# ReaganCardoza/Physics-Based-Ray-Tracing

Hardware: AMD Instinct MI355X
Metric: Msamples/s on cbox.xml 512x512 x 256 spp (radiance, path max_depth 6) (higher is better)
Workload: dtype f32

## Files before the change

### physics-based-ray-tracing_amd/csrc/kernels_radiance.h

```cpp
#pragma once
#include "device_scene.h"
#include "render_request.h"
#include "tile_cull.h"

#ifndef SEG_BRUTE
#define SEG_BRUTE 512
#endif
#ifndef SEG_BVH
#define SEG_BVH 1024
#endif
#ifndef SEG_WAVES_PER_EU
#define SEG_WAVES_PER_EU 8
#endif
#ifndef REGION_SEGS_BVH
#define REGION_SEGS_BVH 4
#endif
#ifndef REGION_SEGS_BRUTE
#define REGION_SEGS_BRUTE 1
#endif
#ifndef REGION_SEGS_US
#define REGION_SEGS_US 8
#endif
__host__ __device__ constexpr uint32_t rad_region_segs(int accel);
#ifndef REGION_SEGS_US_EMIT
// ... 669 lines not shown
#pragma unroll
            for (uint32_t k = 0; k < 2 + MAX_CHAIN; ++k) {
                add[k] = k == 2 ? cnt_in : atomicAdd(&wg_cnt[k < 2 ? k : k - 1], 0u);
                if (k < 2 + nb_run) v[k] = row[k * stride];
            }
#pragma unroll
            for (uint32_t k = 0; k < 2 + MAX_CHAIN; ++k)
                if (k < 2 + nb_run) row[k * stride] = v[k] + add[k];
        }
    }
}

struct TileKeepArgs {
    const pbrt_prim *prims;
    uint32_t n_prims;
    pbrt_camera cam;
    FilmKey key;
    uint32_t n_blocks;
    uint32_t *keep;
};
__global__ __launch_bounds__(64) void k_tile_keep(const TileKeepArgs a) {
    const uint32_t blk = blockIdx.x * 64u + threadIdx.x;
    if (blk >= a.n_blocks) return;
    uint32_t x0 = 0xffffffffu, y0 = 0xffffffffu, x1 = 0, y1 = 0;
    for (uint32_t k = 0; k < 64u; ++k) {
        uint32_t rx, ry;
        region_pixel(a.key, blk * 64u + k, &rx, &ry);
        x0 = min(x0, rx);
        x1 = max(x1, rx);
        y0 = min(y0, ry);
        y1 = max(y1, ry);
    }
    uint32_t word = 0;
    for (uint32_t i = 0; i < a.n_prims && i < 32u; ++i) {
        const pbrt_prim P = load_prim_uniform(a.prims + i);
        if (tile_cull_keep(a.cam, a.key.rx0 + x0, a.key.ry0 + y0, a.key.rx0 + x1, a.key.ry0 + y1, P)) word |= 1u << i;
    }
    word |= a.n_prims < 32u ? ~0u << a.n_prims : 0u;
    a.keep[blk] = word;
}

#define REDUCE_SLICES 32
__global__ __launch_bounds__(256) void k_reduce_stats(const unsigned long long *stats, uint32_t nseg, size_t stride,
                                                      unsigned long long *out) {
    __shared__ unsigned long long part[256];
    const unsigned long long *row = stats + (size_t)blockIdx.x * stride;
    const uint32_t per = (nseg + gridDim.y - 1) / gridDim.y, lo = min(blockIdx.y * per, nseg), hi = min(lo + per, nseg);
    unsigned long long s = 0;
    for (uint32_t i = lo + threadIdx.x; i < hi; i += 256) s += row[i];
    part[threadIdx.x] = s;
    __syncthreads();
    for (uint32_t w = 128; w > 0; w >>= 1) {
        if (threadIdx.x < w) part[threadIdx.x] += part[threadIdx.x + w];
        __syncthreads();
    }
    if (threadIdx.x == 0 && part[0]) atomicAdd(&out[blockIdx.x], part[0]);
}

__global__ __launch_bounds__(256) void k_us_reduce_stats(unsigned long long *stats, uint32_t nseg, size_t stride,
                                                         unsigned long long *out) {
    __shared__ unsigned long long part[4];
    unsigned long long *row = stats + (size_t)blockIdx.x * stride;
    const uint32_t per = (nseg + gridDim.y - 1) / gridDim.y, lo = min(blockIdx.y * per, nseg), hi = min(lo + per, nseg);
    unsigned long long s = 0;
    for (uint32_t i = lo + threadIdx.x; i < hi; i += 256) {
        s += row[i];
        row[i] = 0ull;
    }
#pragma unroll
    for (int off = 32; off > 0; off >>= 1) s += __shfl_xor(s, off);
    if ((threadIdx.x & 63u) == 0u) part[threadIdx.x >> 6] = s;
    __syncthreads();
    if (threadIdx.x == 0) out[(size_t)blockIdx.x * gridDim.y + blockIdx.y] = part[0] + part[1] + part[2] + part[3];
}

struct FilmArgs {
    const float *Lhome;
    float *acc;
    uint32_t cap;
    uint32_t cx0, cy0, cw, ch;
    FilmKey key;
    uint32_t rh;
    uint32_t s_count, filter, seed;
};

DEV float filter_1d(uint32_t f, float x) {
    if (f == PBRT_FILTER_TENT) return fmaxf(0.0f, 1.0f - fabsf(x));
    const float alpha = -2.0f;
    return fmaxf(0.0f, expf(alpha * x * x) - expf(alpha * 4.0f));
}

__global__ __launch_bounds__(256) void k_film_accum(const FilmArgs a) {
    const uint32_t idx = blockIdx.x * blockDim.x + threadIdx.x;
    if (idx >= a.cw * a.ch) return;
    const uint32_t iy = idx / a.cw, ix = idx - iy * a.cw;
    const int x = (int)(a.cx0 + ix), y = (int)(a.cy0 + iy);
    const uint32_t npx = a.cw * a.ch;
    float ar = a.acc[idx], ag = a.acc[npx + idx], ab = a.acc[2 * npx + idx], aw = a.acc[3 * npx + idx];
    const int R = a.filter == PBRT_FILTER_BOX ? 0 : (a.filter == PBRT_FILTER_TENT ? 1 : 2);
    const float ccx = (float)x + 0.5f, ccy = (float)y + 0.5f;
    for (uint32_t sl = 0; sl < a.s_count; ++sl) {
        const uint32_t s_idx = a.key.s_first + sl;
        const float4 *Ls = reinterpret_cast<const float4 *>(a.Lhome) + (size_t)sl * a.key.npix_r;
        for (int ny = y - R; ny <= y + R; ++ny)
            for (int nx = x - R; nx <= x + R; ++nx) {
                if (nx < 0 || ny < 0 || nx >= (int)a.key.film_w || ny >= (int)a.key.film_h) continue;
                float w = 1.0f;
                if (a.filter != PBRT_FILTER_BOX) {
                    F4 uj = rng4((uint32_t)ny * a.key.film_w + (uint32_t)nx, s_idx, 0, a.seed);
                    float px = (float)nx + uj.x, py = (float)ny + uj.y;
                    w = filter_1d(a.filter, ccx - px) * filter_1d(a.filter, ccy - py);
                }
                if (w > 0.0f) {
                    const uint32_t k = region_index((uint32_t)(nx - (int)a.key.rx0), (uint32_t)(ny - (int)a.key.ry0), a.key.rw, a.key.tile_rows);
                    const float4 Lk = Ls[k];
                    ar = fma_(w, Lk.x, ar);
                    ag = fma_(w, Lk.y, ag);
                    ab = fma_(w, Lk.z, ab);
                    aw += w;
                }
            }
    }
    a.acc[idx] = ar;
    a.acc[npx + idx] = ag;
    a.acc[2 * npx + idx] = ab;
    a.acc[3 * npx + idx] = aw;
}

#define FILM_RMAX 2
template <int FILM_TILE, int FILTER>
__global__ __launch_bounds__(FILM_TILE *FILM_TILE) void k_film_accum_tiled(const FilmArgs a) {
    constexpr int FILM_TW = FILM_TILE + 2 * FILM_RMAX;
    constexpr int LS = FILM_TILE == 16 ? 48 : 40;
    static_assert(LS >= FILM_TW, "row stride covers the haloed row");
    __shared__ float tile[2][5][FILM_TW * LS];
    constexpr int R = FILTER == PBRT_FILTER_TENT ? 1 : 2;
    constexpr int TW = FILM_TILE + 2 * R;
    const uint32_t tid = threadIdx.y * FILM_TILE + threadIdx.x;
    const int tx0 = (int)(a.cx0 + blockIdx.x * FILM_TILE), ty0 = (int)(a.cy0 + blockIdx.y * FILM_TILE);
    const int x = tx0 + (int)threadIdx.x, y = ty0 + (int)threadIdx.y;
    const bool inside = x < (int)(a.cx0 + a.cw) && y < (int)(a.cy0 + a.ch);
    const uint32_t npx = a.cw * a.ch;
    const uint32_t idx = inside ? (uint32_t)(y - (int)a.cy0) * a.cw + (uint32_t)(x - (int)a.cx0) : 0u;
    float ar = 0, ag = 0, ab = 0, aw = 0;
    if (inside) {
        ar = a.acc[idx];
        ag = a.acc[npx + idx];
        ab = a.acc[2 * npx + idx];
        aw = a.acc[3 * npx + idx];
    }
    const float ccx = (float)x + 0.5f, ccy = (float)y + 0.5f;
    constexpr int NT = FILM_TILE * FILM_TILE, NST = (FILM_TW * FILM_TW + NT - 1) / NT;
    bool st_in[NST], st_valid[NST];
    uint32_t st_key[NST], st_k[NST];
    float st_x[NST], st_y[NST];
    int st_lds[NST];
#pragma unroll
    for (int j = 0; j < NST; ++j) {
        const int i = (int)tid + j * NT;
        const int nx = tx0 - R + i % TW, ny = ty0 - R + i / TW;
        st_lds[j] = (i / TW) * LS + i % TW;
        st_in[j] = i < TW * TW;
        st_valid[j] = st_in[j] && nx >= (int)a.key.rx0 && ny >= (int)a.key.ry0 && nx < (int)(a.key.rx0 + a.key.rw) && ny < (int)(a.key.ry0 + a.rh);
        st_key[j] = (uint32_t)ny * a.key.film_w + (uint32_t)nx;
        st_k[j] = st_valid[j] ? region_index((uint32_t)(nx - (int)a.key.rx0), (uint32_t)(ny - (int)a.key.ry0), a.key.rw, a.key.tile_rows) : 0u;
        st_x[j] = (float)nx;
        st_y[j] = (float)ny;
    }
    const float4 *Lrec = reinterpret_cast<const float4 *>(a.Lhome);
    const float4 zero4 = {0.0f, 0.0f, 0.0f, 0.0f};
#ifndef FILM_PF
#define FILM_PF 4
#endif
    constexpr int PF = FILM_PF;
    float4 Lq[PF][NST];
#pragma unroll
    for (int u = 0; u < PF; ++u)
#pragma unroll
        for (int j = 0; j < NST; ++j)
            Lq[u][j] = (st_valid[j] && (uint32_t)u < a.s_count) ? Lrec[(size_t)u * a.key.npix_r + st_k[j]] : zero4;
    for (uint32_t sl0 = 0; sl0 < a.s_count; sl0 += PF) {
#pragma unroll
        for (int u = 0; u < PF; ++u) {
            const uint32_t sl = sl0 + (uint32_t)u;
            if (sl >= a.s_count) break;
            const uint32_t s_idx = a.key.s_first + sl;
            float(*T)[FILM_TW * LS] = tile[sl & 1];
#pragma unroll
            for (int j = 0; j < NST; ++j) {
                if (!st_in[j]) continue;
                const int i = st_lds[j];
                float px = 1e30f, py = 1e30f;
                if (st_valid[j]) {
                    F4 uj = rng4(st_key[j], s_idx, 0, a.seed);
                    px = st_x[j] + uj.x;
                    py = st_y[j] + uj.y;
                }
                T[0][i] = px;
                T[1][i] = py;
                T[2][i] = Lq[u][j].x;
                T[3][i] = Lq[u][j].y;
                T[4][i] = Lq[u][j].z;
            }
#pragma unroll
            for (int j = 0; j < NST; ++j)
                Lq[u][j] = (st_valid[j] && sl + PF < a.s_count) ? Lrec[(size_t)(sl + PF) * a.key.npix_r + st_k[j]] : zero4;
            __syncthreads();
            if (inside) {
                const int e0 = (int)threadIdx.y * LS + (int)threadIdx.x;
#pragma unroll
                for (int dy = 0; dy <= 2 * R; ++dy)
#pragma unroll
                    for (int dx = 0; dx <= 2 * R; ++dx) {
                        const int e = e0 + dy * LS + dx;
                        float w = filter_1d(FILTER, ccx - T[0][e]) * filter_1d(FILTER, ccy - T[1][e]);
                        if (w > 0.0f) {
                            ar = fma_(w, T[2][e], ar);
                            ag = fma_(w, T[3][e], ag);
                            ab = fma_(w, T[4][e], ab);
                            aw += w;
                        }
                    }
            }
        }
    }
    if (inside) {
        a.acc[idx] = ar;
        a.acc[npx + idx] = ag;
        a.acc[2 * npx + idx] = ab;
        a.acc[3 * npx + idx] = aw;
    }
}

__global__ __launch_bounds__(256) void k_film_resolve(const float *acc, float *out, uint32_t npx, uint32_t raw) {
    const uint32_t idx = blockIdx.x * blockDim.x + threadIdx.x;
    if (idx >= npx) return;
    float r = acc[idx], g = acc[npx + idx], b = acc[2 * npx + idx], w = acc[3 * npx + idx];
    if (raw) {
        out[4 * idx] = r;
        out[4 * idx + 1] = g;
        out[4 * idx + 2] = b;
        out[4 * idx + 3] = w;
    } else {
        float inv = w > 0.0f ? 1.0f / w : 0.0f;
        out[3 * idx] = r * inv;
        out[3 * idx + 1] = g * inv;
        out[3 * idx + 2] = b * inv;
    }
}

__global__ __launch_bounds__(256) void k_init_rays(float *st, uint32_t *seg_cnt, uint32_t n_cnt, uint32_t region, uint32_t n,
                                                   const float *o, const float *d, const float *tmax) {
    const uint32_t i = blockIdx.x * blockDim.x + threadIdx.x;
    if (i < n_cnt) seg_cnt[i] = n > i * region ? min(n - i * region, region) : 0u;
    if (i >= n) return;
    float *s = st + (state_voff(i) >> 2);
    s[(ST_O + 0) * 64] = o[i];
    s[(ST_O + 1) * 64] = o[n + i];
    s[(ST_O + 2) * 64] = o[2 * n + i];
    s[(ST_D + 0) * 64] = d[i];
    s[(ST_D + 1) * 64] = d[n + i];
    s[(ST_D + 2) * 64] = d[2 * n + i];
    s[(ST_THR + 0) * 64] = 1.0f;
    s[(ST_THR + 1) * 64] = 1.0f;
    s[(ST_THR + 2) * 64] = 1.0f;
    s[(ST_L + 0) * 64] = 0.0f;
    s[(ST_L + 1) * 64] = 0.0f;
    s[(ST_L + 2) * 64] = 0.0f;
    s[ST_ETA * 64] = tmax[i];
    s[ST_PDF * 64] = -1.0f;
    s[ST_HOME * 64] = __uint_as_float(i);
}
```

### physics-based-ray-tracing_amd/csrc/pbrt_api.hip

```cpp
#include <hip/hip_runtime.h>

#include <atomic>
#include <cmath>
#include <cstdarg>
#include <cstdio>
#include <cstring>
#include <map>
#include <numeric>
#include <string>
#include <tuple>
#include <vector>

#include "scene_request.h"
#include "bf_request.h"
#include "us_request.h"
#include "kernels_us.h"
#include "kernels_wavefront.h"
#include "kernels_us_wavefront.h"
#include "kernels_beamform.h"
#ifdef PBRT_DIAG
#include "kernels_diag.h"
#endif
#include "stage_layout.h"
#include "workspace.h"
// ... 844 lines not shown
}
static uint64_t default_pass_paths(pbrt_ctx *c, bool streams, uint64_t paths, uint32_t bytes_per_path) {
    return streams ? wf_default_pass_paths(c) : fused_default_pass_paths(paths, bytes_per_path, c->work.limit);
}

static bool fastdiv_exact(const FastDiv &fd, uint32_t d, std::initializer_list<uint32_t> probes) {
    for (uint32_t n : probes)
        if (udiv_fast(n, fd) != n / d) return false;
    return true;
}

static WfArgs wf_args(const RadArgs &a) {
    WfArgs w{};
    w.sc = a.sc;
    w.cam = a.cam;
    w.Lhome = a.Lhome;
    w.stats = a.stats;
    w.stat_stride = a.stat_stride;
    w.cap = a.cap;
    w.n_paths = a.n_paths;
    w.max_depth = a.max_depth;
    w.rr_depth = a.rr_depth;
    w.seed = a.seed;
    w.key_mode = a.key_mode;
    w.key = a.key;
    w.index_offset = a.index_offset;
    w.sample_index = a.sample_index;
    return w;
}
static void film_accum(pbrt_ctx *c, const FilmArgs &fa) {
    hipStream_t st = c->stream;
    if (fa.filter == PBRT_FILTER_BOX) {
        hipLaunchKernelGGL(k_film_accum, dim3(div_up((uint64_t)fa.cw * fa.ch, 256)), dim3(256), 0, st, fa);
        return;
    }
    const bool big = (uint64_t)div_up(fa.cw, 16) * div_up(fa.ch, 16) >= 4ull * (uint64_t)c->n_cu;
    const bool tent = fa.filter == PBRT_FILTER_TENT;
    const dim3 g16(div_up(fa.cw, 16), div_up(fa.ch, 16)), g8(div_up(fa.cw, 8), div_up(fa.ch, 8));
    if (big && tent)
        hipLaunchKernelGGL((k_film_accum_tiled<16, PBRT_FILTER_TENT>), g16, dim3(16, 16), 0, st, fa);
    else if (big)
        hipLaunchKernelGGL((k_film_accum_tiled<16, PBRT_FILTER_GAUSSIAN>), g16, dim3(16, 16), 0, st, fa);
    else if (tent)
        hipLaunchKernelGGL((k_film_accum_tiled<8, PBRT_FILTER_TENT>), g8, dim3(8, 8), 0, st, fa);
    else
        hipLaunchKernelGGL((k_film_accum_tiled<8, PBRT_FILTER_GAUSSIAN>), g8, dim3(8, 8), 0, st, fa);
}

static int probe_plan(pbrt_ctx *c, unsigned long long *segstats, uint32_t n_rows, uint32_t stat_rows, unsigned long long *dstats,
                      uint32_t max_depth, uint32_t *plan) {
    hipStream_t st = c->stream;
    unsigned long long hp[2 + MAX_DEPTH_STATS];
    hipLaunchKernelGGL(k_reduce_stats, dim3(stat_rows, REDUCE_SLICES), dim3(256), 0, st, segstats, n_rows, (size_t)n_rows, dstats);
    HIPCHK(c, hipGetLastError());
    HIPCHK(c, hipMemcpyAsync(hp, dstats, (size_t)stat_rows * 8, hipMemcpyDeviceToHost, st));
    HIPCHK(c, hipStreamSynchronize(st));
    HIPCHK(c, hipMemsetAsync(dstats, 0, (2 + 2 * MAX_DEPTH_STATS) * 8, st));
    for (uint32_t d = stat_rows; d < 2 + MAX_DEPTH_STATS; ++d) hp[d] = 0;
    *plan = plan_from_survival(hp + 2, std::min<uint32_t>(max_depth, MAX_DEPTH_STATS));
    return PBRT_OK;
}

namespace {
struct Render {
    pbrt_scene *s;
    pbrt_ctx *c;
    const pbrt_camera *cam;
    const pbrt_film_desc *f;
    void *d_out;
    RenderRequest rq;
    Switches sw;
    PassShape ps;
    uint32_t n_own = 0, n_rows = 0;
    WfBufs wfb{};
    WfPlan wfp;
    float *Lhome = nullptr, *acc = nullptr;
    uint32_t *segA = nullptr, *segB = nullptr;
    unsigned long long *dstats = nullptr, *segstats = nullptr;
    FusePlan fp;
    RadArgs base{};
    FilmArgs fa{};
    PassTimer timer{};
    uint32_t passes = 0, launches = 0;
    unsigned long long hstats[2 + 2 * MAX_DEPTH_STATS];
    uint32_t hguard[WF_GUARD_WORDS] = {0};
};
}

static RenderLaunch render_launch(const pbrt_scene *s) {
    static_assert(WF_REGION == REGION_SEGS_BVH * SEG_BVH, "both BVH launch structures cut a pass into the same regions");
    const int k = s->accel_kernel;
    RenderLaunch l;
    l.brute = k == ACCEL_K_BRUTE || k == ACCEL_K_BRUTE_BIG;
    l.keep = k == ACCEL_K_BRUTE && s->ds.n_prims <= 32;
    l.region = rad_region_segs(k) * seg_threads(k);
    l.owners = rad_owners_per_region(k);
    l.rows_fused = k == ACCEL_K_BRUTE ? std::max(rad_rows_per_region(k), path_groups_per_region()) : rad_rows_per_region(k);
    l.rows_streams = WF_SHADE_THREADS / 64u;
    return l;
}

static int render_check(Render &r) {
    pbrt_ctx *c = r.c;
    if (int rcs = ctx_settle(c)) return rcs;
    if (const char *why = render_request(&r.rq, r.cam, r.f, r.d_out != nullptr, render_launch(r.s))) return RULE_TEXT(c, why);
    HIPCHK(c, hipSetDevice(c->device));
    r.sw = read_switches();
    return PBRT_OK;
}

static int render_buffers(Render &r) {
    pbrt_scene *s = r.s;
    pbrt_ctx *c = r.c;
    const pbrt_film_desc *f = r.f;
    const RenderRequest &rq = r.rq;
    const bool wavefront = rq.wavefront;
    const uint64_t pass_paths = f->pass_paths ? f->pass_paths
                                              : default_pass_paths(c, wavefront, rq.brute ? (64u << 20) : (16u << 20), 16 + 2 * N_STATE * 4);
    auto alloc_pass = [&](const PassShape &ps) -> int {
        r.Lhome = (float *)c->buf("Lhome", (size_t)ps.cap * 16);
        return r.Lhome && (!wavefront || wf_alloc(c, ps.cap, ps.nseg, &r.wfb)) ? PBRT_OK : PBRT_E_NOMEM;
    };
    int rc = size_pass(c, pass_paths, f->pass_paths != 0, f->spp, rq.npix_r, rq.launch.region, true, wavefront, N_STATE, alloc_pass, &r.ps);
    if (rc) return rc;
    if (wavefront) {
        r.wfp = wf_plan(s, r.sw);
        if ((rc = wf_set_attr(s, r.wfp)) != 0) return rc;
    }
    r.n_own = r.ps.nseg * rq.launch.owners;
    r.n_rows = r.ps.nseg * rq.rows_per_region();
    r.segA = (uint32_t *)c->buf("segA", (size_t)r.n_own * 4);
    r.segB = (uint32_t *)c->buf("segB", (size_t)r.n_own * 4);
    r.acc = (float *)c->buf("film_acc", rq.film_px * 16);
    r.dstats = (unsigned long long *)c->buf("stats", (2 + 2 * MAX_DEPTH_STATS) * 8);
    r.segstats = (unsigned long long *)c->buf("segstats", (size_t)(2 + 2 * MAX_DEPTH_STATS) * r.n_rows * 8);
    if (!r.segstats) return PBRT_E_NOMEM;
    return r.Lhome && r.segA && r.segB && r.acc && r.dstats ? PBRT_OK : PBRT_E_NOMEM;
}

static int render_clear(Render &r) {
    pbrt_ctx *c = r.c;
    const RenderRequest &rq = r.rq;
    hipStream_t st = c->stream;
    HIPCHK(c, hipMemsetAsync(r.acc, 0, rq.film_px * 16, st));
    HIPCHK(c, hipMemsetAsync(r.dstats, 0, (2 + 2 * MAX_DEPTH_STATS) * 8, st));
    HIPCHK(c, hipMemsetAsync(r.segstats, 0, (size_t)rq.stat_rows * r.n_rows * 8, st));
    if (rq.hit_rows) HIPCHK(c, hipMemsetAsync(r.segstats + (size_t)HIT_ROW0 * r.n_rows, 0, (size_t)rq.hit_rows * r.n_rows * 8, st));
    HIPCHK(c, hipEventRecord(c->ev0, st));
    r.timer = PassTimer{c};
    return PBRT_OK;
}

static void render_plan(Render &r, bool may_probe = true) {
    r.fp = fuse_plan(r.rq, r.s->plan_hint_valid, r.s->plan_hint, r.ps.per_pass, may_probe);
}

static int render_args(Render &r) {
    pbrt_scene *s = r.s;
    const pbrt_film_desc *f = r.f;
    const uint32_t rw = r.rq.rw, cap = r.ps.cap;
    RadArgs &base = r.base;
    base.sc = s->ds;
    if ((f->flags & PBRT_FILM_NO_OCCLUDER_PRUNING) && base.sc.occ_prims) {
        base.sc.occ_prims = base.sc.prims;
        base.sc.n_occ = base.sc.n_prims;
        base.sc.occ_runs = base.sc.prim_runs;
        base.sc.n_occ_runs = base.sc.n_prim_runs;
        base.sc.occ_ord = base.sc.prim_ord;
    }
    if (f->flags & PBRT_FILM_NO_ORDERED_WALK) base.sc.prim_ord = base.sc.occ_ord = 0u;
    base.cam = *r.cam;
    base.Lhome = r.Lhome;
    base.stats = r.segstats;
    base.stat_stride = r.n_rows;
    base.cap = cap;
    base.state_cap = cap;
    base.max_depth = f->max_depth;
    base.rr_depth = f->rr_depth;
    base.seed = f->seed;
    base.key_mode = 0;
    const FilmKey &key = base.key = render_film_key(r.rq);
    const std::initializer_list<uint32_t> probes = {0u, 1u, rw - 1, rw, rw + 1, key.npix_r - 1, key.npix_r, key.npix_r + 1, cap - 1, cap, 0xffffffffu};
    NEED(r.c, fastdiv_exact(key.div_npix, key.npix_r, probes) && fastdiv_exact(key.div_rw, rw, probes));
    base.lds_bytes = s->lds_bytes;
    base.tile_keep = nullptr;
    return PBRT_OK;
}
static void render_film(Render &r) {
    const pbrt_film_desc *f = r.f;
    FilmArgs &fa = r.fa;
    fa.Lhome = r.Lhome;
    fa.acc = r.acc;
    fa.cap = r.ps.cap;
    fa.cx0 = f->crop_x;
    fa.cy0 = f->crop_y;
    fa.cw = f->crop_w;
    fa.ch = f->crop_h;
    fa.key = r.base.key;
    fa.rh = r.rq.rh;
    fa.filter = f->filter;
    fa.seed = f->seed;
}

static int render_tile_keep(Render &r) {
    pbrt_ctx *c = r.c;
    c->tile_keep_last = false;
    if (!r.rq.tile_keep) return PBRT_OK;
    TileKeepArgs ta;
    ta.prims = r.s->ds.prims;
    ta.n_prims = r.s->ds.n_prims;
    ta.cam = *r.cam;
    ta.key = r.base.key;
    ta.n_blocks = ta.key.npix_r / 64;
    ta.keep = (uint32_t *)c->buf("tile_keep", (size_t)ta.n_blocks * 4);
    if (!ta.keep) return PBRT_E_NOMEM;
    const pbrt_ctx::TileKeepKey key{c->work.generation("tile_keep"), r.s->serial, *r.cam, r.rq.rx0, r.rq.ry0, r.rq.rw, r.rq.rh};
    if (!(key == c->tile_keep_key)) {
        hipLaunchKernelGGL(k_tile_keep, dim3(div_up(ta.n_blocks, 64)), dim3(64), 0, c->stream, ta);
        HIPCHK(c, hipGetLastError());
        ++c->tile_keep_builds;
        c->tile_keep_key = key;
    }
    r.base.tile_keep = ta.keep;
    c->tile_keep_last = true;
    c->tile_keep_words = ta.keep;
    return PBRT_OK;
}

static int brute_bounces(pbrt_scene *s, RadArgs a, uint32_t plan, uint32_t nseg_pass, bool camera, uint32_t bound, float *in, float *out,
                         uint32_t *sin, uint32_t *sout, uint32_t n_own, uint32_t *launches, bool path_ok = false) {
    pbrt_ctx *c = s->ctx;
    int rc;
    for (uint32_t depth = 0; depth < a.max_depth && depth < bound;) {
        const uint32_t nb = chain_len(plan, depth, a.max_depth);
        a.depth = depth;
        a.nb = nb;
        a.in = in;
        a.out = out;
        a.seg_in = sin;
        a.seg_out = sout;
        const PathKern whole = path_ok && camera && depth == 0 && nb >= a.max_depth ? path_kernel(s, a.sc.prim_ord != 0u) : nullptr;
        if ((rc = whole ? launch_path(s, whole, a, nseg_pass) : launch_bounce(s, a, nseg_pass, camera && depth == 0, nb)) != 0) return rc;
        HIPCHK(c, hipGetLastError());
        ++*launches;
        std::swap(in, out);
        std::swap(sin, sout);
        const uint32_t depth_before = depth;
        depth += nb;
        bool dead;
        if ((rc = poll_live(c, a.max_depth, depth_before, depth, sin, n_own, &dead)) != 0) return rc;
        if (dead) break;
    }
    return PBRT_OK;
}

constexpr uint32_t PASS_MAX_BOUNCES = 256;
static int brute_pass(Render &r, RadArgs a, uint32_t nseg_pass) {
    pbrt_ctx *c = r.c;
    const uint32_t region = r.rq.launch.region;
    const bool one_launch = chain_len(r.fp.plan, 0, a.max_depth) >= a.max_depth;
    const size_t need = one_launch ? (size_t)region : (size_t)nseg_pass * region;
    float *in = (float *)c->buf("stateA", need * N_STATE * 4), *out = (float *)c->buf("stateB", need * N_STATE * 4);
    if (!in || !out) return PBRT_E_NOMEM;
    a.state_cap = (uint32_t)need;
    if (int rc = r.timer.begin()) return rc;
    return brute_bounces(r.s, a, r.fp.plan, nseg_pass, true, PASS_MAX_BOUNCES, in, out, r.segA, r.segB, r.n_own, &r.launches,
                         !(r.f->flags & PBRT_FILM_NO_PATH_KERNEL));
}

static int render_passes(Render &r) {
    pbrt_ctx *c = r.c;
    const pbrt_film_desc *f = r.f;
    int rc;
    for (PassSchedule p{f->spp, r.ps.per_pass, r.fp.probe}; p.next(); ++r.passes) {
        RadArgs a = r.base;
        a.n_paths = (uint32_t)(r.rq.npix_r * p.sc);
        a.key.s_first = f->sample_offset + p.s0;
        const uint32_t nseg_pass = div_up(a.n_paths, r.rq.launch.region);
        if (r.rq.wavefront) {
            if ((rc = r.timer.begin()) != 0) return rc;
            rc = wf_bounces(r.s, wf_args(a), r.wfb, r.wfp, nseg_pass, true, &r.launches);
        } else {
            rc = brute_pass(r, a, nseg_pass);
        }
        if (rc) return rc;
        if ((rc = r.timer.end()) != 0) return rc;
        r.fa.key.s_first = a.key.s_first;
        r.fa.s_count = p.sc;
        film_accum(c, r.fa);
        HIPCHK(c, hipGetLastError());
        if (p.probing() && (rc = probe_plan(c, r.segstats, r.n_rows, r.rq.stat_rows, r.dstats, f->max_depth, &r.fp.plan)) != 0) return rc;
    }
    return PBRT_OK;
}

static int render_finish(Render &r) {
    pbrt_ctx *c = r.c;
    const RenderRequest &rq = r.rq;
    const uint32_t n_rows = r.n_rows;
    hipStream_t st = c->stream;
    int rc;
    hipLaunchKernelGGL(k_film_resolve, dim3(div_up(rq.film_px, 256)), dim3(256), 0, st, r.acc, (float *)r.d_out, (uint32_t)rq.film_px,
                       (uint32_t)(rq.out_floats == 4 ? 1 : 0));
    HIPCHK(c, hipGetLastError());
    HIPCHK(c, hipEventRecord(c->ev1, st));
    hipLaunchKernelGGL(k_reduce_stats, dim3(rq.stat_rows, REDUCE_SLICES), dim3(256), 0, st, r.segstats, n_rows, (size_t)n_rows, r.dstats);
    if (rq.hit_rows)
        hipLaunchKernelGGL(k_reduce_stats, dim3(rq.hit_rows, REDUCE_SLICES), dim3(256), 0, st, r.segstats + (size_t)HIT_ROW0 * n_rows, n_rows,
                           (size_t)n_rows, r.dstats + HIT_ROW0);
    HIPCHK(c, hipGetLastError());
    HIPCHK(c, hipMemcpyAsync(r.hstats, r.dstats, sizeof r.hstats, hipMemcpyDeviceToHost, st));
    if (rq.wavefront && (rc = wf_guard_fetch(c, r.hguard)) != 0) return rc;
    HIPCHK(c, hipStreamSynchronize(st));
    return rq.wavefront ? wf_check_guard(c, r.hguard) : PBRT_OK;
}

static int render_stats(Render &r) {
    pbrt_ctx *c = r.c;
    const unsigned long long *hstats = r.hstats;
    if (int rc = call_stats(c, hstats, r.rq.npix_r * r.f->spp, r.launches, r.passes, true, r.timer.n_ev)) return rc;
    pbrt_stats &S = c->stats;
    S.fuse_plan = r.fp.plan;
    S.plan_source = r.fp.source;
    S.pass_paths = (uint64_t)r.rq.npix_r * r.ps.per_pass;
    if (r.rq.brute && hstats[2] > 0) {
        r.s->plan_hint = plan_from_survival(hstats + 2, (uint32_t)std::min<uint64_t>(r.f->max_depth, MAX_DEPTH_STATS));
        r.s->plan_hint_valid = true;
    }
    const ModelBytes m = render_model_bytes(r.rq, hstats, S.samples, r.passes, r.fp.plan);
    S.model_bytes = m.total;
    S.bounce_model_bytes = m.bounce;
    if (r.rq.wavefront) S.trace_model_bytes = m.trace;
    return PBRT_OK;
}

#ifdef PBRT_DIAG
#include "diag_driver.h"
#endif

static int render_impl(pbrt_scene *s, const pbrt_camera *cam, const pbrt_film_desc *f, void *d_out) {
    Render r{s, s->ctx, cam, f, d_out};
    int rc;
    if ((rc = render_check(r)) != 0) return rc;
#ifdef PBRT_DIAG
    if (diag_selected(r)) return diag_render(r);
#else
    if ((f->flags & (PBRT_FILM_REGEN | PBRT_FILM_WALK_SET)) || (!r.rq.brute && (f->flags & PBRT_FILM_NO_HIT_POOL)))
        return r.c->fail(PBRT_E_UNSUPPORTED, "PBRT_FILM_REGEN / PBRT_FILM_WALK_FROM / PBRT_FILM_NO_HIT_POOL select diagnostic launch "
                                             "structures: build libpbrt_hip_diag.so (make -C csrc diag)");
#endif
    if ((rc = render_buffers(r)) != 0) return rc;
    if ((rc = render_clear(r)) != 0) return rc;
    render_plan(r);
    if ((rc = render_args(r)) != 0) return rc;
    if ((rc = render_tile_keep(r)) != 0) return rc;
    render_film(r);
    if ((rc = render_passes(r)) != 0) return rc;
    if ((rc = render_finish(r)) != 0) return rc;
    return render_stats(r);
}

#ifdef PBRT_BVH_PROBE
extern "C" int pbrt_debug_bvh_probe(unsigned long long *out, int reset) {
    if (out && hipMemcpyFromSymbol(out, HIP_SYMBOL(g_bvh_probe), 64) != hipSuccess) return PBRT_E_DEVICE;
    if (reset) {
        unsigned long long z[8] = {0, 0, 0, 0, 0, 0, 0, 0};
        if (hipMemcpyToSymbol(HIP_SYMBOL(g_bvh_probe), z, 64) != hipSuccess) return PBRT_E_DEVICE;
    }
    return PBRT_OK;
}
#endif

namespace {
struct SampleCall {
    pbrt_scene *s;
    pbrt_ctx *c;
    uint32_t n;
    const float *o, *d, *tmax;
    uint32_t index_offset, sample_index, seed, max_depth, rr_depth;
    float *rgb;
    Switches sw;
    RenderLaunch launch;
    bool streams = false;
    PassShape ps;
    uint32_t n_own = 0, n_rows = 0;
    WfBufs wfb{};
    WfPlan wfp;
    float *stA = nullptr, *stB = nullptr, *Lhome = nullptr, *dO = nullptr, *dD = nullptr, *dT = nullptr;
    uint32_t *segA = nullptr, *segB = nullptr;
    unsigned long long *dstats = nullptr, *rows = nullptr;
    size_t rows_bytes = 0;
    RadArgs a{};
    uint32_t hguard[WF_GUARD_WORDS] = {0};
};
}

static int sample_check(SampleCall &q) {
    pbrt_ctx *c = q.c;
    HIPCHK(c, hipSetDevice(c->device));
    if (int rcs = ctx_settle(c)) return rcs;
    ++c->call_seq;
    q.sw = read_switches();
    q.launch = render_launch(q.s);
    q.streams = !q.launch.brute;
    return one_pass(c, q.n, 1, q.n, q.launch.region, false, q.streams, N_STATE, &q.ps);
}

static int sample_buffers(SampleCall &q) {
    pbrt_scene *s = q.s;
    pbrt_ctx *c = q.c;
    const uint32_t cap = q.ps.cap, nseg = q.ps.nseg;
    q.n_own = nseg * q.launch.owners;
    if (q.streams) {
        if (!wf_alloc(c, cap, nseg, &q.wfb)) return PBRT_E_NOMEM;
        q.wfp = wf_plan(s, q.sw);
        if (int rc = wf_set_attr(s, q.wfp)) return rc;
    } else {
        q.stA = (float *)c->buf("stateA", (size_t)cap * N_STATE * 4);
        q.stB = (float *)c->buf("stateB", (size_t)cap * N_STATE * 4);
        q.segA = (uint32_t *)c->buf("segA", (size_t)q.n_own * 4);
        q.segB = (uint32_t *)c->buf("segB", (size_t)q.n_own * 4);
        q.dstats = (unsigned long long *)c->buf("stats", (2 + MAX_DEPTH_STATS) * 8);
        if (!q.stA || !q.stB || !q.segA || !q.segB || !q.dstats) return PBRT_E_NOMEM;
    }
    q.Lhome = (float *)c->buf("Lhome", (size_t)cap * 16);
    q.n_rows = nseg * (q.streams ? q.launch.rows_streams : q.launch.rows_fused);
    q.rows_bytes = (size_t)(2 + (q.streams ? 2 : 1) * MAX_DEPTH_STATS) * q.n_rows * 8;
    q.rows = (unsigned long long *)c->buf("segstats", q.rows_bytes);
    const size_t n = q.n;
    const auto io_at = stage_layout(stage_in(q.o, 3 * n), stage_in(q.d, 3 * n), stage_in(q.tmax, n));
    char *io = (char *)c->buf("leaf_io", io_at.total);
    if (!q.Lhome || !q.rows || !io) return PBRT_E_NOMEM;
    q.dO = (float *)(io + io_at.offset[0]);
// ... 1235 lines not shown
```

### physics-based-ray-tracing_amd/csrc/render_request.h

```cpp
#pragma once
#include <algorithm>
#include <cstddef>
#include <cstdint>

#include "../../include/pbrt_hip.h"
#include "film_key.h"

#define N_STATE 15
#define MAX_DEPTH_STATS 62
#define MAX_CHAIN 6
#define HIT_ROW0 (2 + MAX_DEPTH_STATS)

static inline uint32_t div_up(uint64_t a, uint64_t b) { return (uint32_t)((a + b - 1) / b); }

#define RENDER_RULE(cond)          \
    do {                           \
        if (!(cond)) return #cond; \
    } while (0)

struct RenderLaunch {
    bool brute;
    bool keep;
    uint32_t region;
    uint32_t owners;
// ... 61 lines not shown
struct PassShape {
    uint32_t per_pass = 1, cap = 0, nseg = 0;
};
static inline const char *pass_shape(PassShape *ps, uint64_t pass_paths, uint32_t per_call, uint64_t unit, uint32_t region, bool equal) {
    uint32_t k = (uint32_t)std::max<uint64_t>(1, std::min<uint64_t>(per_call, pass_paths / std::max<uint64_t>(unit, 1)));
    if (equal) k = div_up(per_call, div_up(per_call, k));
    RENDER_RULE(unit * k < 0xfffffc00ull);
    ps->per_pass = k;
    ps->cap = div_up(unit * k, region) * region;
    ps->nseg = ps->cap / region;
    return nullptr;
}
static inline bool pass_halve(uint64_t *pass_paths, bool fixed, const PassShape &ps, uint64_t unit) {
    if (fixed || ps.per_pass <= 1 || *pass_paths <= PASS_MIN_PATHS) return false;
    *pass_paths = std::max<uint64_t>(PASS_MIN_PATHS, std::min<uint64_t>(*pass_paths, unit * ps.per_pass) / 2);
    return true;
}
static inline const char *pass_addressing(uint32_t cap, bool wavefront, uint32_t rows, uint32_t dead) {
    if (!(wavefront || (uint64_t)cap * rows * 4 < 0xffffffffull)) return "wavefront || (uint64_t)cap * N_STATE * 4 < 0xffffffffull";
    if (wavefront && !(cap < dead)) return "cap < WF_DEAD";
    return nullptr;
}

static inline uint64_t stream_default_pass_paths(size_t free_b, size_t total_b, size_t held, size_t limit, size_t ws_total,
                                                 uint32_t bytes_per_path) {
    double budget = std::min((2.0 / 3.0) * (double)(free_b + held), 0.5 * (double)total_b);
    if (limit) budget = std::min(budget, (double)limit - (double)(ws_total - held) - 64e6 );
    uint64_t pass_paths = PASS_MIN_PATHS;
    while (pass_paths < (512u << 20) && 2.0 * (double)pass_paths * bytes_per_path <= budget) pass_paths *= 2;
    return pass_paths;
}
static inline uint64_t fused_default_pass_paths(uint64_t paths, uint32_t bytes_per_path, size_t limit) {
    if (limit)
        while (paths > PASS_MIN_PATHS && (double)paths * (double)bytes_per_path > (double)limit - 64e6) paths /= 2;
    return paths;
}

#ifndef PBRT_DEFAULT_FUSE_PLAN
#define PBRT_DEFAULT_FUSE_PLAN 0x15u
#endif
static inline uint32_t chain_len(uint32_t plan, uint32_t depth, uint32_t max_depth) {
    uint32_t nb = 1;
    while (nb < MAX_CHAIN && depth + nb < max_depth && depth + nb - 1 < 32 && ((plan >> (depth + nb - 1)) & 1u)) ++nb;
    return nb;
}
static inline uint32_t plan_from_survival(const unsigned long long *live, uint32_t max_depth) {
    uint32_t plan = 0;
    for (uint32_t d = 0; d + 1 < max_depth && d < 31; ++d) {
        const bool last = d + 2 == max_depth;
        if (live[d] == 0) break;
        if (last || (double)live[d + 1] >= 0.45 * (double)live[d]) plan |= 1u << d;
    }
    return plan;
}
constexpr uint32_t PROBE_SPP = 2;
struct FusePlan {
    uint32_t plan = 0;
    bool probe = false;
    uint32_t source = PBRT_PLAN_DEFAULT;
};
static inline FusePlan fuse_plan(const RenderRequest &rq, bool hint_valid, uint32_t hint, uint32_t s_pass, bool may_probe = true) {
    const uint32_t flags = rq.f->flags;
    const bool caller = (flags & PBRT_FILM_FUSE_PLAN_SET) != 0, learnt = rq.brute && hint_valid;
    FusePlan p;
    p.plan = !rq.brute ? 0u : caller ? ((flags >> 8) & 0xffu) : (hint_valid ? hint : PBRT_DEFAULT_FUSE_PLAN);
    p.probe = may_probe && rq.brute && !hint_valid && rq.f->spp >= 8 * PROBE_SPP && s_pass >= PROBE_SPP && !caller;
    p.source = rq.wavefront ? PBRT_PLAN_STREAMS : caller ? PBRT_PLAN_CALLER : p.probe ? PBRT_PLAN_PROBED : learnt ? PBRT_PLAN_LEARNT : PBRT_PLAN_DEFAULT;
    return p;
}
struct PassSchedule {
    uint32_t spp, s_pass;
    bool probe;
    uint32_t s0 = 0, sc = 0, passes = 0;
    bool probing() const { return probe && passes == 1; }
    bool next() {
        s0 += sc;
        if (s0 >= spp) return false;
        if (probing()) s_pass = div_up(spp - s0, div_up(spp - s0, s_pass));
        sc = probe && passes == 0 ? PROBE_SPP : std::min(s_pass, spp - s0);
        ++passes;
        return true;
    }
};

struct WfShape {
    uint32_t threads, rows;
    size_t lds;
    bool packet;
};
static inline WfShape wf_shape(uint32_t lds_limit, uint32_t image, uint32_t bvh_depth, bool packet) {
    WfShape p;
    const uint32_t limit = lds_limit ? lds_limit : 65536u;
    p.threads = 1024u;
    const uint32_t statics = 1024;
    uint32_t budget = limit / 2;
    if (image + statics + 3u * p.threads * 4u > budget) budget = limit;
    const uint32_t rows_fit = (budget - image - statics) / (p.threads * 4u);
    p.rows = std::max(2u, std::min(rows_fit, 8u));
    p.packet = packet && 3u * bvh_depth <= 64u;
    p.lds = (size_t)image + (size_t)p.rows * p.threads * 4u;
    return p;
}
static inline uint32_t wf_trace_grid(uint32_t nr, uint32_t mult, uint32_t cus, uint32_t kmax) {
    return std::min(nr, std::max(div_up(nr, kmax), std::max(1u, mult * cus)));
}
static inline void wf_part(uint32_t nreg, uint32_t parts, uint32_t h, uint32_t *reg0, uint32_t *regn) {
    *reg0 = (uint32_t)((uint64_t)nreg * h / parts);
    *regn = (uint32_t)((uint64_t)nreg * (h + 1) / parts) - *reg0;
}

static inline void radiance_model_bytes(const unsigned long long *live, uint32_t nd, uint64_t samples, uint64_t film_px,
                                        uint32_t passes, uint32_t fuse_plan, uint32_t max_depth, const unsigned long long *hits,
                                        uint64_t *total, uint64_t *bounce) {
    uint64_t b = 0;
    for (uint32_t d = 0; d < nd;) {
        const uint32_t nb = std::min(chain_len(fuse_plan, d, max_depth), nd - d);
        uint64_t in = live[d], next = (d + nb < nd) ? live[d + nb] : 0;
        if (d > 0 && hits)
            b += in * 24 + hits[d] * (N_STATE * 4);
        else if (d > 0)
            b += in * (N_STATE * 4);
        b += next * (N_STATE * 4);
        b += (in - next) * 12;
        d += nb;
    }
    *bounce = b;
    *total = b + samples * 12  + film_px * 32ull * passes  +
             film_px * 28 ;
}
static inline uint64_t wavefront_model_bytes(const unsigned long long *live, const unsigned long long *hits, uint32_t nd, uint64_t shadows,
                                             uint64_t *trace) {
    uint64_t tr = 0, sh = 0;
    for (uint32_t d = 0; d < nd; ++d) {
        const uint64_t in = live[d], next = d + 1 < nd ? live[d + 1] : 0, h = std::min<uint64_t>(hits[d], in);
        if (!in) break;
        tr += (d > 0 ? in * 32 : 0) + in * 4;
        sh += in * 4 + (d > 0 ? (in - h) * 48 + h * 96 : 0);
        sh += (in - next) * 16 + next * 96;
    }
    tr += shadows * 36;
    sh += shadows * 32;
    if (trace) *trace = tr;
    return tr + sh;
}
struct ModelBytes {
    uint64_t total, bounce, trace;
};
static inline ModelBytes render_model_bytes(const RenderRequest &rq, const unsigned long long *hstats, uint64_t samples, uint32_t passes,
                                            uint32_t plan) {
    ModelBytes m{0, 0, 0};
    radiance_model_bytes(hstats + 2, MAX_DEPTH_STATS, samples, rq.film_px, passes, plan, rq.f->max_depth,
                         rq.wavefront ? hstats + HIT_ROW0 : nullptr, &m.total, &m.bounce);
    if (rq.wavefront) {
        m.total -= m.bounce;
        m.bounce = wavefront_model_bytes(hstats + 2, hstats + HIT_ROW0, MAX_DEPTH_STATS, hstats[1], &m.trace);
        m.total += m.bounce;
    }
    return m;
}
```

Measured before the change: 11790.

## Fuse film clear and resolve into gather pass; batch two samples per LDS tile

The film accumulation kernel now skips reading the accumulator on the first pass and writes the resolved output directly on the last pass. This removes the accumulator memset and the separate resolve kernel. The tiled kernel now stages two samples per synchronisation step, packed side by side in one LDS row, instead of double-buffering one sample with a deep prefetch queue. It also uses branchless accumulation and a launch bound sized for four workgroups per CU. The risks are correctness when a render has a single pass or uses edge tiles, and the extra barrier added per batch.

```diff
diff --git a/physics-based-ray-tracing_amd/csrc/kernels_radiance.h b/physics-based-ray-tracing_amd/csrc/kernels_radiance.h
--- a/physics-based-ray-tracing_amd/csrc/kernels_radiance.h
+++ b/physics-based-ray-tracing_amd/csrc/kernels_radiance.h
@@ -775,12 +775,44 @@
     FilmKey key;
     uint32_t rh;
     uint32_t s_count, filter, seed;
+    bool first, last;
+    uint32_t out_floats;
+    float *out;
 };
 
 DEV float filter_1d(uint32_t f, float x) {
     if (f == PBRT_FILTER_TENT) return fmaxf(0.0f, 1.0f - fabsf(x));
     const float alpha = -2.0f;
     return fmaxf(0.0f, expf(alpha * x * x) - expf(alpha * 4.0f));
+}
+
+DEV void film_resolve_px(float *out, uint32_t idx, bool raw, float r, float g, float b, float w) {
+    if (raw) {
+        out[4 * idx] = r;
+        out[4 * idx + 1] = g;
+        out[4 * idx + 2] = b;
+        out[4 * idx + 3] = w;
+    } else {
+        float inv = w > 0.0f ? 1.0f / w : 0.0f;
+        out[3 * idx] = r * inv;
+        out[3 * idx + 1] = g * inv;
+        out[3 * idx + 2] = b * inv;
+    }
+}
+DEV void film_sums_in(const FilmArgs &a, uint32_t idx, uint32_t npx, float &ar, float &ag, float &ab, float &aw) {
+    ar = ag = ab = aw = 0.0f;
+    if (a.first) return;
+    ar = a.acc[idx];
+    ag = a.acc[npx + idx];
+    ab = a.acc[2 * npx + idx];
+    aw = a.acc[3 * npx + idx];
+}
+DEV void film_sums_out(const FilmArgs &a, uint32_t idx, uint32_t npx, float ar, float ag, float ab, float aw) {
+    if (a.last) return film_resolve_px(a.out, idx, a.out_floats == 4, ar, ag, ab, aw);
+    a.acc[idx] = ar;
+    a.acc[npx + idx] = ag;
+    a.acc[2 * npx + idx] = ab;
+    a.acc[3 * npx + idx] = aw;
 }
 
 __global__ __launch_bounds__(256) void k_film_accum(const FilmArgs a) {
@@ -789,7 +821,8 @@
     const uint32_t iy = idx / a.cw, ix = idx - iy * a.cw;
     const int x = (int)(a.cx0 + ix), y = (int)(a.cy0 + iy);
     const uint32_t npx = a.cw * a.ch;
-    float ar = a.acc[idx], ag = a.acc[npx + idx], ab = a.acc[2 * npx + idx], aw = a.acc[3 * npx + idx];
+    float ar, ag, ab, aw;
+    film_sums_in(a, idx, npx, ar, ag, ab, aw);
     const int R = a.filter == PBRT_FILTER_BOX ? 0 : (a.filter == PBRT_FILTER_TENT ? 1 : 2);
     const float ccx = (float)x + 0.5f, ccy = (float)y + 0.5f;
     for (uint32_t sl = 0; sl < a.s_count; ++sl) {
@@ -814,21 +847,19 @@
                 }
             }
     }
-    a.acc[idx] = ar;
-    a.acc[npx + idx] = ag;
-    a.acc[2 * npx + idx] = ab;
-    a.acc[3 * npx + idx] = aw;
-}
-
-#define FILM_RMAX 2
+    film_sums_out(a, idx, npx, ar, ag, ab, aw);
+}
+
+constexpr int FILM_B = 2;
 template <int FILM_TILE, int FILTER>
-__global__ __launch_bounds__(FILM_TILE *FILM_TILE) void k_film_accum_tiled(const FilmArgs a) {
-    constexpr int FILM_TW = FILM_TILE + 2 * FILM_RMAX;
-    constexpr int LS = FILM_TILE == 16 ? 48 : 40;
-    static_assert(LS >= FILM_TW, "row stride covers the haloed row");
-    __shared__ float tile[2][5][FILM_TW * LS];
+__global__ __launch_bounds__(FILM_TILE *FILM_TILE, FILM_TILE == 16 ? 4 : 1) void k_film_accum_tiled(const FilmArgs a) {
+    constexpr int B = FILM_B;
     constexpr int R = FILTER == PBRT_FILTER_TENT ? 1 : 2;
-    constexpr int TW = FILM_TILE + 2 * R;
+    constexpr int TW = FILM_TILE + 2 * R, NE = TW * TW;
+    constexpr int LS = FILM_TILE == 16 ? 48 : 40, HALF = LS / 2;
+    static_assert(B % 2 == 0 && HALF >= TW, "a row holds the haloed rows of two images");
+    static_assert(FILM_TILE != 16 || (B / 2) * 5 * TW * LS * 4 <= 40960, "four workgroups of the 16-pixel instances per CU");
+    __shared__ float tile[B / 2][5][TW * LS];
     const uint32_t tid = threadIdx.y * FILM_TILE + threadIdx.x;
     const int tx0 = (int)(a.cx0 + blockIdx.x * FILM_TILE), ty0 = (int)(a.cy0 + blockIdx.y * FILM_TILE);
     const int x = tx0 + (int)threadIdx.x, y = ty0 + (int)threadIdx.y;
@@ -836,24 +867,20 @@
     const uint32_t npx = a.cw * a.ch;
     const uint32_t idx = inside ? (uint32_t)(y - (int)a.cy0) * a.cw + (uint32_t)(x - (int)a.cx0) : 0u;
     float ar = 0, ag = 0, ab = 0, aw = 0;
-    if (inside) {
-        ar = a.acc[idx];
-        ag = a.acc[npx + idx];
-        ab = a.acc[2 * npx + idx];
-        aw = a.acc[3 * npx + idx];
-    }
+    if (inside) film_sums_in(a, idx, npx, ar, ag, ab, aw);
     const float ccx = (float)x + 0.5f, ccy = (float)y + 0.5f;
-    constexpr int NT = FILM_TILE * FILM_TILE, NST = (FILM_TW * FILM_TW + NT - 1) / NT;
-    bool st_in[NST], st_valid[NST];
-    uint32_t st_key[NST], st_k[NST];
-    float st_x[NST], st_y[NST];
-    int st_lds[NST];
-#pragma unroll
-    for (int j = 0; j < NST; ++j) {
-        const int i = (int)tid + j * NT;
+    constexpr int NT = FILM_TILE * FILM_TILE, NSB = (B * NE + NT - 1) / NT;
+    bool st_in[NSB], st_valid[NSB];
+    uint32_t st_key[NSB], st_k[NSB], st_u[NSB];
+    float st_x[NSB], st_y[NSB];
+    int st_lds[NSB];
+#pragma unroll
+    for (int j = 0; j < NSB; ++j) {
+        const int e = (int)tid + j * NT, u = e / NE, i = e % NE;
         const int nx = tx0 - R + i % TW, ny = ty0 - R + i / TW;
-        st_lds[j] = (i / TW) * LS + i % TW;
-        st_in[j] = i < TW * TW;
+        st_in[j] = e < B * NE;
+        st_u[j] = (uint32_t)u;
+        st_lds[j] = st_in[j] ? (u / 2) * 5 * TW * LS + (i / TW) * LS + (u % 2) * HALF + i % TW : 0;
         st_valid[j] = st_in[j] && nx >= (int)a.key.rx0 && ny >= (int)a.key.ry0 && nx < (int)(a.key.rx0 + a.key.rw) && ny < (int)(a.key.ry0 + a.rh);
         st_key[j] = (uint32_t)ny * a.key.film_w + (uint32_t)nx;
         st_k[j] = st_valid[j] ? region_index((uint32_t)(nx - (int)a.key.rx0), (uint32_t)(ny - (int)a.key.ry0), a.key.rw, a.key.tile_rows) : 0u;
@@ -861,85 +888,62 @@
         st_y[j] = (float)ny;
     }
     const float4 *Lrec = reinterpret_cast<const float4 *>(a.Lhome);
-    const float4 zero4 = {0.0f, 0.0f, 0.0f, 0.0f};
-#ifndef FILM_PF
-#define FILM_PF 4
-#endif
-    constexpr int PF = FILM_PF;
-    float4 Lq[PF][NST];
-#pragma unroll
-    for (int u = 0; u < PF; ++u)
-#pragma unroll
-        for (int j = 0; j < NST; ++j)
-            Lq[u][j] = (st_valid[j] && (uint32_t)u < a.s_count) ? Lrec[(size_t)u * a.key.npix_r + st_k[j]] : zero4;
-    for (uint32_t sl0 = 0; sl0 < a.s_count; sl0 += PF) {
-#pragma unroll
-        for (int u = 0; u < PF; ++u) {
-            const uint32_t sl = sl0 + (uint32_t)u;
-            if (sl >= a.s_count) break;
-            const uint32_t s_idx = a.key.s_first + sl;
-            float(*T)[FILM_TW * LS] = tile[sl & 1];
-#pragma unroll
-            for (int j = 0; j < NST; ++j) {
-                if (!st_in[j]) continue;
-                const int i = st_lds[j];
+    float4 Lq[NSB];
+#pragma unroll
+    for (int j = 0; j < NSB; ++j) Lq[j] = Lrec[(st_valid[j] && st_u[j] < a.s_count) ? (size_t)st_u[j] * a.key.npix_r + st_k[j] : (size_t)0];
+    float *const T0 = &tile[0][0][0];
+    const int e0 = (int)threadIdx.y * LS + (int)threadIdx.x;
+    for (uint32_t sl0 = 0; sl0 < a.s_count; sl0 += B) {
+#pragma unroll
+        for (int j = 0; j < NSB; ++j) {
+            const uint32_t sl = sl0 + st_u[j];
+            if (st_in[j]) {
+                float *Tj = T0 + st_lds[j];
                 float px = 1e30f, py = 1e30f;
-                if (st_valid[j]) {
-                    F4 uj = rng4(st_key[j], s_idx, 0, a.seed);
+                if (st_valid[j] && sl < a.s_count) {
+                    F4 uj = rng4(st_key[j], a.key.s_first + sl, 0, a.seed);
                     px = st_x[j] + uj.x;
                     py = st_y[j] + uj.y;
                 }
-                T[0][i] = px;
-                T[1][i] = py;
-                T[2][i] = Lq[u][j].x;
-                T[3][i] = Lq[u][j].y;
-                T[4][i] = Lq[u][j].z;
+                Tj[0] = px;
+                Tj[TW * LS] = py;
+                Tj[2 * TW * LS] = Lq[j].x;
+                Tj[3 * TW * LS] = Lq[j].y;
+                Tj[4 * TW * LS] = Lq[j].z;
             }
-#pragma unroll
-            for (int j = 0; j < NST; ++j)
-                Lq[u][j] = (st_valid[j] && sl + PF < a.s_count) ? Lrec[(size_t)(sl + PF) * a.key.npix_r + st_k[j]] : zero4;
-            __syncthreads();
-            if (inside) {
-                const int e0 = (int)threadIdx.y * LS + (int)threadIdx.x;
+            Lq[j] = Lrec[(st_valid[j] && sl + B < a.s_count) ? (size_t)(sl + B) * a.key.npix_r + st_k[j] : (size_t)0];
+        }
+        __syncthreads();
+        if (inside) {
+#pragma unroll
+            for (int u = 0; u < B; ++u) {
+                if (sl0 + (uint32_t)u >= a.s_count) break;
+                const float(*T)[TW * LS] = tile[u / 2];
 #pragma unroll
                 for (int dy = 0; dy <= 2 * R; ++dy)
 #pragma unroll
                     for (int dx = 0; dx <= 2 * R; ++dx) {
-                        const int e = e0 + dy * LS + dx;
-                        float w = filter_1d(FILTER, ccx - T[0][e]) * filter_1d(FILTER, ccy - T[1][e]);
-                        if (w > 0.0f) {
-                            ar = fma_(w, T[2][e], ar);
-                            ag = fma_(w, T[3][e], ag);
-                            ab = fma_(w, T[4][e], ab);
-                            aw += w;
-                        }
+                        const int e = e0 + dy * LS + (u % 2) * HALF + dx;
+                        const float w = filter_1d(FILTER, ccx - T[0][e]) * filter_1d(FILTER, ccy - T[1][e]);
+                        const float Lr = T[2][e], Lg = T[3][e], Lb = T[4][e];
+                        const float nr = fma_(w, Lr, ar), ng = fma_(w, Lg, ag), nb = fma_(w, Lb, ab), nw = aw + w;
+                        const bool on = w > 0.0f;
+                        ar = on ? nr : ar;
+                        ag = on ? ng : ag;
+                        ab = on ? nb : ab;
+                        aw = on ? nw : aw;
                     }
             }
         }
-    }
-    if (inside) {
-        a.acc[idx] = ar;
-        a.acc[npx + idx] = ag;
-        a.acc[2 * npx + idx] = ab;
-        a.acc[3 * npx + idx] = aw;
-    }
+        __syncthreads();
+    }
+    if (inside) film_sums_out(a, idx, npx, ar, ag, ab, aw);
 }
 
 __global__ __launch_bounds__(256) void k_film_resolve(const float *acc, float *out, uint32_t npx, uint32_t raw) {
     const uint32_t idx = blockIdx.x * blockDim.x + threadIdx.x;
     if (idx >= npx) return;
-    float r = acc[idx], g = acc[npx + idx], b = acc[2 * npx + idx], w = acc[3 * npx + idx];
-    if (raw) {
-        out[4 * idx] = r;
-        out[4 * idx + 1] = g;
-        out[4 * idx + 2] = b;
-        out[4 * idx + 3] = w;
-    } else {
-        float inv = w > 0.0f ? 1.0f / w : 0.0f;
-        out[3 * idx] = r * inv;
-        out[3 * idx + 1] = g * inv;
-        out[3 * idx + 2] = b * inv;
-    }
+    film_resolve_px(out, idx, raw != 0u, acc[idx], acc[npx + idx], acc[2 * npx + idx], acc[3 * npx + idx]);
 }
 
 __global__ __launch_bounds__(256) void k_init_rays(float *st, uint32_t *seg_cnt, uint32_t n_cnt, uint32_t region, uint32_t n,
diff --git a/physics-based-ray-tracing_amd/csrc/pbrt_api.hip b/physics-based-ray-tracing_amd/csrc/pbrt_api.hip
--- a/physics-based-ray-tracing_amd/csrc/pbrt_api.hip
+++ b/physics-based-ray-tracing_amd/csrc/pbrt_api.hip
@@ -950,6 +950,7 @@
     FilmArgs fa{};
     PassTimer timer{};
     uint32_t passes = 0, launches = 0;
+    bool gather_flags = false;
     unsigned long long hstats[2 + 2 * MAX_DEPTH_STATS];
     uint32_t hguard[WF_GUARD_WORDS] = {0};
 };
@@ -1010,7 +1011,7 @@
     pbrt_ctx *c = r.c;
     const RenderRequest &rq = r.rq;
     hipStream_t st = c->stream;
-    HIPCHK(c, hipMemsetAsync(r.acc, 0, rq.film_px * 16, st));
+    if (!r.gather_flags) HIPCHK(c, hipMemsetAsync(r.acc, 0, rq.film_px * 16, st));
     HIPCHK(c, hipMemsetAsync(r.dstats, 0, (2 + 2 * MAX_DEPTH_STATS) * 8, st));
     HIPCHK(c, hipMemsetAsync(r.segstats, 0, (size_t)rq.stat_rows * r.n_rows * 8, st));
     if (rq.hit_rows) HIPCHK(c, hipMemsetAsync(r.segstats + (size_t)HIT_ROW0 * r.n_rows, 0, (size_t)rq.hit_rows * r.n_rows * 8, st));
@@ -1068,6 +1069,9 @@
     fa.rh = r.rq.rh;
     fa.filter = f->filter;
     fa.seed = f->seed;
+    fa.first = fa.last = false;
+    fa.out_floats = r.rq.out_floats;
+    fa.out = (float *)r.d_out;
 }
 
 static int render_tile_keep(Render &r) {
@@ -1155,6 +1159,8 @@
         if ((rc = r.timer.end()) != 0) return rc;
         r.fa.key.s_first = a.key.s_first;
         r.fa.s_count = p.sc;
+        r.fa.first = r.gather_flags && gather_flags(p).first;
+        r.fa.last = r.gather_flags && gather_flags(p).last;
         film_accum(c, r.fa);
         HIPCHK(c, hipGetLastError());
         if (p.probing() && (rc = probe_plan(c, r.segstats, r.n_rows, r.rq.stat_rows, r.dstats, f->max_depth, &r.fp.plan)) != 0) return rc;
@@ -1168,8 +1174,9 @@
     const uint32_t n_rows = r.n_rows;
     hipStream_t st = c->stream;
     int rc;
-    hipLaunchKernelGGL(k_film_resolve, dim3(div_up(rq.film_px, 256)), dim3(256), 0, st, r.acc, (float *)r.d_out, (uint32_t)rq.film_px,
-                       (uint32_t)(rq.out_floats == 4 ? 1 : 0));
+    if (!r.gather_flags)
+        hipLaunchKernelGGL(k_film_resolve, dim3(div_up(rq.film_px, 256)), dim3(256), 0, st, r.acc, (float *)r.d_out, (uint32_t)rq.film_px,
+                           (uint32_t)(rq.out_floats == 4 ? 1 : 0));
     HIPCHK(c, hipGetLastError());
     HIPCHK(c, hipEventRecord(c->ev1, st));
     hipLaunchKernelGGL(k_reduce_stats, dim3(rq.stat_rows, REDUCE_SLICES), dim3(256), 0, st, r.segstats, n_rows, (size_t)n_rows, r.dstats);
@@ -1217,6 +1224,7 @@
         return r.c->fail(PBRT_E_UNSUPPORTED, "PBRT_FILM_REGEN / PBRT_FILM_WALK_FROM / PBRT_FILM_NO_HIT_POOL select diagnostic launch "
                                              "structures: build libpbrt_hip_diag.so (make -C csrc diag)");
 #endif
+    r.gather_flags = true;
     if ((rc = render_buffers(r)) != 0) return rc;
     if ((rc = render_clear(r)) != 0) return rc;
     render_plan(r);
diff --git a/physics-based-ray-tracing_amd/csrc/render_request.h b/physics-based-ray-tracing_amd/csrc/render_request.h
--- a/physics-based-ray-tracing_amd/csrc/render_request.h
+++ b/physics-based-ray-tracing_amd/csrc/render_request.h
@@ -167,6 +167,10 @@
         return true;
     }
 };
+struct GatherFlags {
+    bool first, last;
+};
+static inline GatherFlags gather_flags(const PassSchedule &p) { return {p.passes == 1, p.s0 + p.sc >= p.spp}; }
 
 struct WfShape {
     uint32_t threads, rows;
```

Result: no change. 11880 (median of 6 runs) (+0.7%).
